# PreferredAI/cornac

Hardware: AMD Instinct MI355X
Metric: bpr_triplets_per_sec (higher is better)
Workload: dtype f32

## Files before the change

cornac_amd/csrc/bpr.hip:

```cpp
#include <algorithm>
#include <numeric>
#include <queue>

#include "common.h"
#include "rng.h"
#include "sgd_device.h"

namespace chip {

__global__ __launch_bounds__(kBlock) void bpr_det_sample_kernel(
    const uint32_t *__restrict__ pos_draw, int pos_stride, const uint32_t *__restrict__ neg_draw, int neg_stride,
    int64_t n, const int32_t *__restrict__ user_ids, const int32_t *__restrict__ indices,
    const int32_t *__restrict__ indptr, int neg_population, int32_t *__restrict__ su, int32_t *__restrict__ si,
    int32_t *__restrict__ sj, unsigned long long *__restrict__ counters) {
    const int64_t s = (int64_t)blockIdx.x * kBlock + threadIdx.x;
    bool skip = false;
    if (s < n) {
        const uint32_t ii = pos_draw[s * pos_stride];
        const uint32_t jj = neg_draw[s * neg_stride];
        const int32_t u = user_ids[ii];
        const int32_t i = indices[ii];
        const int32_t j = neg_population == CORNAC_HIP_NEG_POPULARITY ? indices[jj] : (int32_t)jj;
        skip = csr_row_contains(indices, indptr[u], indptr[u + 1], j);
        su[s] = skip ? -1 : u;
        si[s] = i;
        sj[s] = j;
    }
    const unsigned long long m = __ballot(skip);
    if (lane_id() == 0 && m) atomicAdd(&counters[1], (unsigned long long)__popcll(m));
}

template <int G, class T>
__global__ __launch_bounds__(kBlock) void bpr_det_level_kernel(const int32_t *__restrict__ su,
                                                               const int32_t *__restrict__ si,
                                                               const int32_t *__restrict__ sj, int64_t off, int cnt,
                                                               T *U, T *V, T *B, int k, T lr,
                                                               T reg, int use_bias,
                                                               unsigned long long *__restrict__ counters) {
    const int gid = (blockIdx.x * kBlock + threadIdx.x) / G;
    const int lg = threadIdx.x & (G - 1);
    const bool active = gid < cnt;
    const int64_t t = off + (active ? gid : cnt - 1);
    const int32_t u = su[t], i = si[t], j = sj[t];
    T *pu = U + (size_t)u * k, *pi = V + (size_t)i * k, *pj = V + (size_t)j * k;
    const T bi = B[i], bj = B[j];
    T score = bi - bj;
    constexpr int RMAX = 4;
    T ru[RMAX], ri[RMAX], rj[RMAX];
    const bool in_regs = k <= RMAX * G;
#pragma unroll
    for (int r = 0; r < RMAX; ++r) {
        const int f = r * G + lg;
        ru[r] = ri[r] = rj[r] = T(0);
        if (in_regs && f < k) {
            ru[r] = pu[f];
            ri[r] = pi[f];
            rj[r] = pj[f];
        }
    }
    auto ordered_add = [&](T p, int lim) { score = ordered_lane_sum_t<G>(score, p, lim); };
    if (in_regs) {
#pragma unroll
        for (int r = 0; r < RMAX; ++r) {
            const int base = r * G;
            if (base < k) ordered_add(base + lg < k ? ru[r] * (ri[r] - rj[r]) : T(0), min(G, k - base));
        }
    } else {
        for (int base = 0; base < k; base += G) {
            const int f = base + lg;
            ordered_add(f < k ? pu[f] * (pi[f] - pj[f]) : T(0), min(G, k - base));
        }
    }
    const T z = sigmoid_neg_exact_t(score);
    if (active) {
        if (in_regs) {
#pragma unroll
            for (int r = 0; r < RMAX; ++r) {
                const int f = r * G + lg;
                if (f < k) {
                    const T uf = ru[r], vi = ri[r], vj = rj[r];
                    pu[f] = uf + lr * (z * (vi - vj) - reg * uf);
                    pi[f] = vi + lr * (z * uf - reg * vi);
                    pj[f] = vj + lr * (-z * uf - reg * vj);
                }
            }
// ... 1404 lines not shown
    const int grid = di.cus * h->strata_blocks_per_cu;
    const int64_t W = (int64_t)grid * kWavesPerBlock;
    if (h->own_waves != W) h->strata_built = false;
    build_ownership(h, W);
    build_item_ranks(h);
    h->rec_u.ensure((size_t)h->nnz);
    h->rec_i.ensure((size_t)h->nnz);
    h->sptr.ensure((size_t)W * 8 + 1);
    REQUIRE(grid % 8 == 0, "the strata grid must be a multiple of the 8 XCDs");
    h->strata_claim.ensure(8 * 16);
    return grid;
}

static void strata_build_buckets(cornac_hip_bpr_t h, int grid, uint32_t key) {
    if (h->strata_built && h->strata_key_built == key) return;
    StrataArgs s;
    s.own_u = h->own_u.p; s.own_i = h->own_i.p; s.wave_ptr = h->wave_ptr.p; s.item_rank = h->item_rank.p;
    s.rec_u = h->rec_u.p; s.rec_i = h->rec_i.p; s.sptr = h->sptr.p;
    s.key = key; s.n_hot = h->strata_n_hot; s.n_waves = (int64_t)grid * kWavesPerBlock;
    h->strata_own_code.ensure((size_t)h->nnz);
    s.own_code = h->strata_own_code.p;
    if (h->strata_code_waves != h->own_waves) {
        hipLaunchKernelGGL(strata_code_kernel, dim3((unsigned)std::min<int64_t>(4096, (h->nnz + kBlock - 1) / kBlock)),
                           dim3(kBlock), 0, h->stream, s, h->nnz);
        h->strata_code_waves = h->own_waves;
    }
    hipLaunchKernelGGL(strata_bucket_kernel, dim3(grid), dim3(kBlock), 0, h->stream, s);
    HIP_CHECK(hipGetLastError());
    h->strata_built = true;
    h->strata_key_built = key;
    ++h->strata_builds;
}

static void strata_enqueue(cornac_hip_bpr_t h, int64_t n_samples, float lr, float reg, int use_bias, int flags) {
    const int grid = strata_prepare(h);
    const bool packed = h->strata_allow_pack && ((h->V.owned && h->B.owned) || h->chunk_records) &&
                        !prof_env_set("CORNAC_HIP_STRATA_NO_PACK");
    if (packed) strata_pack(h); else strata_unpack(h);
    if (!packed) h->Bpad.ensure((size_t)h->total_items * kBiasStride);
    const unsigned bgrid = (unsigned)((h->total_items + kBlock - 1) / kBlock);
    int64_t left = n_samples;
    while (left > 0) {
        const int64_t n = std::min(left, h->nnz - h->hog_offset);
        const auto first_phase = [&](int64_t s) { return (int)((8 * (__int128)s + h->nnz - 1) / h->nnz); };
        const int p_lo = first_phase(h->hog_offset), p_hi = h->hog_offset + n >= h->nnz ? 8 : first_phase(h->hog_offset + n);
        if (p_hi > p_lo) {
            uint32_t key = strata_key(h->hog_seed, h->hog_epoch / (uint32_t)std::max(1, h->strata_rehash_period));
            if (prof_env_int("CORNAC_HIP_STRATA_CONTIG", 0)) key = 0x12345u;
            strata_build_buckets(h, grid, key);
            HogArgs a;
            fill_hog_args(h, a, h->nnz, lr, reg, use_bias, CORNAC_HIP_NEG_UNIFORM, flags);
            const bool dense_bias = !packed && prof_env_int("CORNAC_HIP_STRATA_DENSE_BIAS", 0) != 0;
            a.B = dense_bias ? h->B.p : h->Bpad.p;
            a.bstride = dense_bias ? 1 : kBiasStride;
            if (packed) {
                a.V = h->VB.p;
                a.vpitch = h->vb_pitch;
                a.B = h->VB.p + h->vb_kp;
                a.bstride = h->vb_pitch;
            }
            a.rec_u = h->rec_u.p; a.rec_i = h->rec_i.p; a.rank_item = h->rank_item.p; a.sptr = h->sptr.p;
            a.strata_key = key; a.n_hot = h->strata_n_hot;
            HIP_CHECK(hipMemsetAsync(h->strata_claim.p, 0, 8 * 16 * sizeof(uint32_t), h->stream));
            if (!dense_bias && !packed)
                hipLaunchKernelGGL(bias_pad_kernel, dim3(bgrid), dim3(kBlock), 0, h->stream, h->B.p, h->Bpad.p, h->total_items);
            for (int ph = p_lo; ph < p_hi; ++ph) {
                a.phase = ph;
                a.xcd_claim = h->strata_claim.p + 16 * ph;
                h->ktimer.before(h->stream);
                hipLaunchKernelGGL(h->strata_kernel, dim3(grid), dim3(kBlock), 0, h->stream, a);
                h->ktimer.after(h->stream);
            }
            if (!dense_bias && !packed)
                hipLaunchKernelGGL(bias_unpad_kernel, dim3(bgrid), dim3(kBlock), 0, h->stream, h->Bpad.p, h->B.p, h->total_items);
            HIP_CHECK(hipGetLastError());
        }
        advance_hog_offset(h, n);
        left -= n;
    }
}

typedef void (*LdsBinKernel)(const LdsBinArgs);
constexpr int kLdsbinPresampleDefault = 0;
static LdsBinKernel pick_ldsbin_kernel(int k, bool pop, bool exch = false, bool passing = false, bool conv = false, bool pre = false) {
    if (pre) {
        if (k <= 64) return bpr_ldsbin_kernel<1, 4, false, false, 1, false, true>;
        return bpr_ldsbin_kernel<2, 2, false, false, 1, false, true>;
    }
    if (conv) {
        if (pop) {
            if (k <= 64) return bpr_ldsbin_kernel<1, 4, true, false, 1, true>;
            if (k <= 128) return bpr_ldsbin_kernel<2, 4, true, false, 1, true>;
            if (k <= 192) return bpr_ldsbin_kernel<3, 2, true, false, 1, true>;
            return bpr_ldsbin_kernel<4, 1, true, false, 1, true>;
        }
        if (k <= 64) return bpr_ldsbin_kernel<1, 4, false, false, 1, true>;
        if (k <= 128) return bpr_ldsbin_kernel<2, 4, false, false, 1, true>;
        if (k <= 192) return bpr_ldsbin_kernel<3, 2, false, false, 1, true>;
        return bpr_ldsbin_kernel<4, 1, false, false, 1, true>;
    }
    if (passing && !exch && k > 64 && k <= 128) {
#ifdef CORNAC_PROFILE
        if (prof_env_int("CORNAC_HIP_LDSBIN_UNR", 0) == 0)
#endif
            return pop ? bpr_ldsbin_kernel<2, 4, true> : bpr_ldsbin_kernel<2, 4>;
    }
    if (exch) {
        if (pop) {
            if (k <= 64) return bpr_ldsbin_kernel<1, 4, true, true>;
            if (k <= 128) return bpr_ldsbin_kernel<2, 2, true, true>;
            if (k <= 192) return bpr_ldsbin_kernel<3, 2, true, true>;
            return bpr_ldsbin_kernel<4, 1, true, true>;
        }
        if (k <= 64) return bpr_ldsbin_kernel<1, 4, false, true>;
        if (k <= 128) return bpr_ldsbin_kernel<2, 2, false, true>;
        if (k <= 192) return bpr_ldsbin_kernel<3, 2, false, true>;
        return bpr_ldsbin_kernel<4, 1, false, true>;
    }
    if (pop) {
        if (k <= 64) return bpr_ldsbin_kernel<1, 4, true>;
        if (k <= 128) return bpr_ldsbin_kernel<2, 2, true>;
        if (k <= 192) return bpr_ldsbin_kernel<3, 2, true>;
        return bpr_ldsbin_kernel<4, 1, true>;
    }
#ifdef CORNAC_PROFILE
    if (k <= 64) switch (prof_env_int("CORNAC_HIP_LDSBIN_UNR", 0)) {
        case 1: return bpr_ldsbin_kernel<1, 1>;
        case 2: return bpr_ldsbin_kernel<1, 2>;
        case 8: return bpr_ldsbin_kernel<1, 8>;
        default: break;
    }
    else if (k <= 128) switch (prof_env_int("CORNAC_HIP_LDSBIN_UNR", 0)) {
        case 3: return bpr_ldsbin_kernel<2, 3>;
        case 4: return bpr_ldsbin_kernel<2, 4>;
        case 22: return bpr_ldsbin_kernel<2, 2, false, false, 2>;
        case 32: return bpr_ldsbin_kernel<2, 3, false, false, 2>;
        case 42: return bpr_ldsbin_kernel<2, 4, false, false, 2>;
        default: break;
    }
#endif
    if (k <= 64) return bpr_ldsbin_kernel<1, 4>;
    if (k <= 128) return bpr_ldsbin_kernel<2, 2>;
    if (k <= 192) return bpr_ldsbin_kernel<3, 2>;
    return bpr_ldsbin_kernel<4, 1>;
}

constexpr size_t kLbLdsBudget = 96 * 1024;
constexpr size_t kLbLdsExclusive = 82 * 1024;
static size_t ldsbin_lds_bytes(int cap, int k, int waves = kLbWaves) {
    const int kp = ((k + kWave - 1) / kWave) * kWave;
    return ((size_t)cap * (kp + 5) + 1) * sizeof(float) + (size_t)waves * 3 * kWave * sizeof(int32_t);
}

struct LbPlan {
    int bins = 0, block = kLbBlock, cap = 0;
    size_t lds = 0;
    bool passing = false;
};
static LbPlan ldsbin_plan(cornac_hip_bpr_t h) {
    LbPlan pl;
    const int cus = device_info(h->device).cus;
    if (h->cv_blocks) {
        if (h->k > 256) return pl;
        const int waves = h->lb_pass_waves;
        const size_t budget = (size_t)h->lb_pass_kb << 10;
        const int kp = ((h->k + kWave - 1) / kWave) * kWave;
        const size_t fixed = sizeof(float) + (size_t)waves * 3 * kWave * sizeof(int32_t);
        if (budget <= fixed) return pl;
        const int64_t cap_lds = (int64_t)((budget - fixed) / ((size_t)(kp + 5) * sizeof(float)));
        const int64_t cap_min = std::max<int64_t>(h->lb_min_candidates, 16);
        if (cap_lds < cap_min) return pl;
        int64_t bins = (h->n_items + cap_lds - 1) / cap_lds;
        const int64_t more = std::min<int64_t>(h->n_items / (cap_min + cap_min / 3), (int64_t)2 * cus * h->cv_blocks);
        bins = std::max(bins, more);
        bins = std::max<int64_t>(1, (bins + h->cv_blocks - 1) / h->cv_blocks) * h->cv_blocks;
        const int64_t cap = (h->n_items + bins - 1) / bins;
        if (cap > cap_lds || bins > (int64_t(1) << 22) || bins * cap >= (int64_t(1) << 31)) return pl;
        pl.bins = (int)bins;
        pl.cap = (int)cap;
        pl.block = waves * kWave;
        pl.lds = ldsbin_lds_bytes((int)cap, h->k, waves);
        pl.passing = true;
        return pl;
    }
    if (h->k > 256 || h->nnz < (int64_t)cus * kLbWaves * kWave) return pl;
    const int res_waves = prof_env_int("CORNAC_HIP_LDSBIN_RES_WAVES", kLbWaves);
    for (int rounds = prof_env_int("CORNAC_HIP_LDSBIN_MIN_ROUNDS", 1); rounds <= h->lb_max_rounds; ++rounds) {
        const int64_t bins = (int64_t)cus * rounds;
        const int64_t cap = (h->n_items + bins - 1) / bins;
        if (cap < h->lb_min_candidates) return pl;
        if (ldsbin_lds_bytes((int)cap, h->k, res_waves) <= (size_t)prof_env_int("CORNAC_HIP_LDSBIN_BUDGET_KB", (int)(kLbLdsBudget >> 10)) << 10) {
            pl.bins = (int)bins;
            pl.cap = (int)cap;
            pl.block = res_waves * kWave;
            pl.lds = std::max(ldsbin_lds_bytes((int)cap, h->k, res_waves), (size_t)prof_env_int("CORNAC_HIP_LDSBIN_EXCL_KB", (int)(kLbLdsExclusive >> 10)) << 10);
            return pl;
        }
    }
    if (!h->lb_pass_enable || (double)h->nnz * 100.0 < (double)h->n_items * h->lb_pass_min_draws_x100) return pl;
    const int waves = prof_env_int("CORNAC_HIP_LDSBIN_PASS_WAVES", h->lb_pass_waves);
    const size_t budget = (size_t)prof_env_int("CORNAC_HIP_LDSBIN_PASS_KB", h->lb_pass_kb) << 10;
    const int kp = ((h->k + kWave - 1) / kWave) * kWave;
    const size_t fixed = sizeof(float) + (size_t)waves * 3 * kWave * sizeof(int32_t);
    if (budget <= fixed) return pl;
    int64_t cap = (int64_t)((budget - fixed) / ((size_t)(kp + 5) * sizeof(float)));
    if (cap < h->lb_min_candidates) return pl;
    int64_t bins = (h->n_items + cap - 1) / cap;
    bins = ((bins + cus - 1) / cus) * cus;
    cap = (h->n_items + bins - 1) / bins;
    if (cap < h->lb_min_candidates || bins > (int64_t(1) << 22)) return pl;
    pl.bins = (int)bins;
    pl.cap = (int)cap;
    pl.block = waves * kWave;
    pl.lds = ldsbin_lds_bytes((int)cap, h->k, waves);
    pl.passing = true;
    return pl;
}

static bool ldsbin_can_run(cornac_hip_bpr_t h, int64_t n_samples, int neg_population) {
    if (neg_population == CORNAC_HIP_NEG_POPULARITY && h->neg_pop_n) return false;
    const LbPlan pl = ldsbin_plan(h);
    return pl.bins > 0 && (!pl.passing || n_samples * 4 >= h->nnz);
}

static void ldsbin_build(cornac_hip_bpr_t h) {
    const LbPlan plan = ldsbin_plan(h);
    const int bins = plan.bins;
    if (h->lb_built && h->lb_bins == bins && h->lb_block == plan.block && h->lb_lds_bytes == plan.lds) return;
// ... 766 lines not shown
```

cornac_amd/csrc/bpr_ldsbin.inc:

```


namespace chip {

constexpr int kLbBlock = 1024;
constexpr int kLbWaves = kLbBlock / kWave;
constexpr int32_t kLbHot = (int32_t)0x80000000;
constexpr int kLbMaxExchanges = 32;
constexpr int kLbMaxRanges = 8;

struct LdsBinExchange {
    float *base;
    float *bucket;
    float *keep;
    unsigned int *arrive;
    const unsigned int *landed;
    unsigned int *applied;
    long long bucket_stride, keep_stride;
    long long nt;
    int n_ex, rule;
};

struct LdsBinArgs {
    const int32_t *cptr, *cusers;
    const int32_t *rank_item;
// ... 316 lines not shown
        uint32_t run = 0;
        for (uint32_t g0 = 0; g0 < n_groups; g0 += kWave) {
            const uint32_t g = g0 + lane;
            uint32_t v = g < n_groups ? cum[g + 1] : 0u;
#pragma unroll
            for (int o = 1; o < kWave; o <<= 1) {
                const uint32_t t = __shfl_up(v, o, kWave);
                if (lane >= o) v += t;
            }
            if (g < n_groups) cum[g + 1] = run + v;
            run += __shfl(v, kWave - 1, kWave);
        }
        if (lane == 0) {
            cum[0] = 0;
            *sh_next_tile = 0;
            *sh_cold_mass = run;
            *sh_nslots = (n_groups && item[n_groups - 1] == -1) ? n_groups - 1 : n_groups;
        }
    }
    __syncthreads();
}

template <bool POP>
__device__ __forceinline__ LdsBinDraw ldsbin_draw(const LdsBinArgs &a, const LdsBinCtx &c, uint32_t local, bool in_range) {
    LdsBinDraw d;
    d.in_range = in_range;
    uint32_t w[4];
    philox4x32_10(d.in_range ? local : 0u, c.b, a.epoch, 0x20u, (uint32_t)a.seed, (uint32_t)(a.seed >> 32), w);
    const uint32_t r_pos = lemire_bounded2(w[0], w[1], c.n_draws, c.th_draw);
    uint32_t s_j, excl = 0, excl_lo = 0xffffffffu;
    if (r_pos < c.cold_mass) {
        uint32_t lo = 0, hi = c.n_slots;
        while (hi - lo > 1) {
            const uint32_t mid = (lo + hi) >> 1;
            if (c.cum[mid] <= r_pos) lo = mid; else hi = mid;
        }
        d.u = a.cusers[c.cp[lo] + (int32_t)(r_pos - c.cum[lo])];
        d.ei = (int32_t)lo;
        s_j = c.n_slots > 1 ? lemire_bounded2(w[2], w[3], c.n_slots - 1, c.th_slot1) : 0u;
        if (c.n_slots > 1 && s_j >= lo) ++s_j;
        excl_lo = c.cum[lo];
        excl = c.cum[lo + 1] - excl_lo;
    } else {
        const uint32_t h = c.hot_lo + (r_pos - c.cold_mass);
        d.u = a.hot_u[h];
        d.ei = a.hot_i[h] | kLbHot;
        s_j = lemire_bounded2(w[2], w[3], c.n_slots, c.th_slot);
    }
    if (POP) {
        const uint32_t m = c.n_draws - excl;
        uint32_t r_neg = (uint32_t)(((uint64_t)w[2] * m) >> 32);
        if (r_neg >= excl_lo) r_neg += excl;
        if (m == 0) {
            d.j = c.item[d.ei] & ~kLbHot;
            d.ej = d.ei;
        } else if (r_neg < c.cold_mass) {
            uint32_t lo = 0, hi = c.n_slots;
            while (hi - lo > 1) {
                const uint32_t mid = (lo + hi) >> 1;
                if (c.cum[mid] <= r_neg) lo = mid; else hi = mid;
            }
            d.j = c.item[lo];
            d.ej = (int32_t)lo;
        } else {
            d.j = a.hot_i[c.hot_lo + (r_neg - c.cold_mass)];
            d.ej = d.j | kLbHot;
        }
        return d;
    }
    const int32_t itj = c.item[s_j];
    d.j = itj & ~kLbHot;
    d.ej = itj < 0 ? itj : (int32_t)s_j;
    return d;
}

__device__ __forceinline__ void ldsbin_launch_range(const LdsBinArgs &a, uint32_t n_draws, uint32_t n_waves, uint32_t &d_lo,
                                                    uint32_t &d_hi, uint32_t &tile_w, uint32_t &n_tiles) {
    d_lo = (uint32_t)(((unsigned __int128)n_draws * a.s_begin) / a.nnz);
    d_hi = a.s_begin + a.n >= a.nnz ? n_draws : (uint32_t)(((unsigned __int128)n_draws * (a.s_begin + a.n)) / a.nnz);
    tile_w = (d_hi - d_lo) < 8u * n_waves * kWave ? 32u : 64u;
    n_tiles = (d_hi - d_lo + tile_w - 1) / tile_w;
}

template <int R, int UNR, bool POP = false, bool EXCH = false, int PF = 1, bool CONV = false, bool PRE = false>
__global__ __launch_bounds__(kLbBlock) void bpr_ldsbin_kernel(const LdsBinArgs a) {
    constexpr int G = kWave, KP = G * R, NREF = 2 * UNR;
    extern __shared__ float lb_smem[];
    float *const rows = lb_smem;
    float *const bias = rows + (size_t)a.cap * KP;
    int32_t *const item = reinterpret_cast<int32_t *>(bias + a.cap);
    int32_t *const cp = item + a.cap;
    uint32_t *const cum = reinterpret_cast<uint32_t *>(cp + a.cap);
    int *const lock = reinterpret_cast<int *>(cum + a.cap + 1);
    int32_t(*const stage)[3][kWave] = reinterpret_cast<int32_t(*)[3][kWave]>(lock + a.cap);
    const int wave = threadIdx.x >> 6, lane = lane_id();
    const uint32_t n_waves = blockDim.x >> 6;
    uint32_t b = blockIdx.x;
    const uint32_t nb = (uint32_t)a.n_bins;
    float *cvV = nullptr, *cvB = nullptr;
    if (CONV) {
        const uint32_t r = blockIdx.x / (uint32_t)a.conv_bpb, o = blockIdx.x - r * (uint32_t)a.conv_bpb;
        b = (uint32_t)a.conv_first[r] + o;
        cvV = a.conv_rows[r] + (size_t)o * (size_t)a.cap * (size_t)a.k;
        cvB = a.conv_rows[r] + (size_t)a.conv_bpb * (size_t)a.cap * (size_t)a.k + (size_t)o * (size_t)a.cap;
    }
    const uint32_t n_groups = ((uint32_t)a.n_items + nb - 1) / nb;
#ifdef CORNAC_PROFILE
    if (a.wg_clock && threadIdx.x == 0) a.wg_clock[2 * b] = wall_clock64();
#endif
    __shared__ uint32_t sh_nslots, sh_cold_mass, sh_next_tile;
    __shared__ uint32_t sh_ex_done[kLbMaxExchanges], sh_ex_applied[kLbWaves];
    __shared__ int sh_ex_lock[kLbWaves];
    if (EXCH) {
        if (threadIdx.x < kLbMaxExchanges) sh_ex_done[threadIdx.x] = 0;
        if (threadIdx.x < kLbWaves) {
            sh_ex_applied[threadIdx.x] = 0;
            sh_ex_lock[threadIdx.x] = 0;
        }
    }
    ldsbin_build_tables(a, b, nb, n_groups, item, cp, cum, lock, &sh_nslots, &sh_cold_mass, &sh_next_tile);
    const uint32_t n_slots = sh_nslots, cold_mass = sh_cold_mass;
    const uint32_t hot_lo = a.hot_off[b], hot_share = a.hot_off[b + 1] - hot_lo;
    const uint32_t n_draws = n_slots ? cold_mass + hot_share : 0u;
    const uint32_t th_draw = n_draws ? lemire_thresh(n_draws) : 0u, th_slot = n_slots ? lemire_thresh(n_slots) : 0u,
                   th_slot1 = n_slots > 1 ? lemire_thresh(n_slots - 1) : 0u;
    bool inb[R];
#pragma unroll
    for (int r = 0; r < R; ++r) inb[r] = lane + G * r < a.k;
    {
        constexpr int NL = R <= 2 ? 4 : 2;
        for (uint32_t s0 = wave; s0 < n_slots; s0 += n_waves * NL) {
            float t[NL][R], tb[NL];
            int32_t its[NL];
#pragma unroll
            for (int q = 0; q < NL; ++q) {
                const uint32_t sq = s0 + (uint32_t)q * n_waves;
                its[q] = sq < n_slots ? item[sq] : -1;
                const size_t it = (size_t)(its[q] >= 0 ? its[q] : 0);
                const float *pv = CONV ? cvV + (size_t)(its[q] >= 0 ? sq : 0u) * a.k : a.V + it * a.k;
                const float *pb = CONV ? cvB + (its[q] >= 0 ? sq : 0u) : a.B + it;
#pragma unroll
                for (int r = 0; r < R; ++r) t[q][r] = (its[q] >= 0 && inb[r]) ? pv[lane + G * r] : 0.f;
                tb[q] = (its[q] >= 0 && lane == 0) ? *pb : 0.f;
            }
#pragma unroll
            for (int q = 0; q < NL; ++q) {
                if (its[q] < 0) continue;
                const uint32_t sq = s0 + (uint32_t)q * n_waves;
#pragma unroll
                for (int r = 0; r < R; ++r) rows[(size_t)sq * KP + lane + G * r] = t[q][r];
                if (lane == 0) bias[sq] = tb[q];
            }
        }
    }
    __syncthreads();
    unsigned int n_correct = 0, n_skipped = 0;
    if (!PRE && n_slots == 0 && wave == 0 && lane == 0 && a.s_begin == 0) n_skipped = cold_mass + hot_share;
    uint32_t d_lo, d_hi, tile_w, n_tiles;
    ldsbin_launch_range(a, n_draws, n_waves, d_lo, d_hi, tile_w, n_tiles);
    const LdsBinCtx ctx{item, cp, cum, b, n_slots, cold_mass, hot_lo, n_draws, th_draw, th_slot, th_slot1};
    typedef LdsBinDraw Draws;
    auto draw_tile = [&](uint32_t tile) {
        const uint32_t local = d_lo + tile * tile_w + lane;
        return ldsbin_draw<POP>(a, ctx, local, tile < n_tiles && (uint32_t)lane < tile_w && local < d_hi);
    };
    auto member_word = [&](const Draws &d) -> uint32_t {
        return (a.bitmap && !LB_ABLATE(1)) ? a.bitmap[(size_t)d.u * a.bm_words + (d.j >> 5)] : 0u;
    };
    auto member_bounds = [&](const Draws &d, int32_t &lo, int32_t &hi) {
        lo = hi = 0;
        if (!a.bitmap && !LB_ABLATE(1) && d.in_range) {
            lo = a.indptr[d.u];
            hi = a.indptr[d.u + 1];
        }
    };
    auto claim_tile = [&]() -> uint32_t {
        uint32_t t = 0;
        if (lane == 0) t = atomicAdd(&sh_next_tile, 1u);
        return (uint32_t)__builtin_amdgcn_readfirstlane((int)t);
    };
    const uint32_t ex_per = EXCH ? n_tiles / (uint32_t)a.ex.n_ex : 0u;
    const uint32_t ex_parts = ex_per < n_waves ? ex_per : n_waves;
    auto ex_landed_upto = [&](int from, int below) -> int {
        int e = from;
        if (lane == 0)
            while (e < below && __hip_atomic_load(a.ex.landed + e, __ATOMIC_RELAXED, __HIP_MEMORY_SCOPE_SYSTEM) != 0u) ++e;
        return __builtin_amdgcn_readfirstlane(e);
    };
    auto ex_duty = [&](uint32_t t) {
        if (!EXCH || ex_parts == 0u || t >= n_tiles) return;
        const uint32_t q = t / ex_per, part = t - q * ex_per;
        if (q == 0u || q >= (uint32_t)a.ex.n_ex || part >= ex_parts) return;
        const int e = (int)q - 1;
        if (lane == 0)
            while (atomicCAS(&sh_ex_lock[part], 0, 1) != 0) __builtin_amdgcn_s_sleep(2);
        __builtin_amdgcn_fence(__ATOMIC_ACQUIRE, "workgroup");
        const int e_lo = (int)sh_ex_applied[part];
        const int e_hi = ex_landed_upto(e_lo, e);
        if (e_hi > e_lo) __builtin_amdgcn_fence(__ATOMIC_ACQUIRE, "agent");
        constexpr int NB = R == 1 ? 4 : 2;
        if (!LB_ABLATE(64)) {
            for (uint32_t s = part; s < n_slots; s += ex_parts) {
                const int32_t it = item[s];
                if (it >= 0)
                    ex_row_duty<R>(a.ex, a.V, a.B, a.k, it, rows + (size_t)s * KP, bias + s, lock + s, e_lo, e_hi, e, lane, inb, a.counters + 3);
            }
        } else
        for (uint32_t s0 = part; s0 < n_slots; s0 += ex_parts * NB) {
            int32_t its[NB];
            float *lrow[NB], *lbias[NB];
            int *llock[NB];
#pragma unroll
            for (int q = 0; q < NB; ++q) {
                const uint32_t s = s0 + (uint32_t)q * ex_parts;
                const uint32_t sc = s < n_slots ? s : s0;
                const int32_t it = item[sc];
                its[q] = (s < n_slots && it >= 0) ? it : -1;
                lrow[q] = rows + (size_t)sc * KP;
                lbias[q] = bias + sc;
                llock[q] = lock + sc;
            }
            ex_rows_duty<R, NB>(a.ex, a.k, its, lrow, lbias, llock, e_lo, e_hi, e, lane, inb, a.counters + 3);
        }
        if (part == 0u)
            for (uint32_t hr = b; hr < (uint32_t)a.n_hot; hr += nb)
                ex_row_duty<R>(a.ex, a.V, a.B, a.k, a.rank_item[hr], nullptr, nullptr, nullptr, e_lo, e_hi, e, lane, inb, a.counters + 3);
        asm volatile("s_waitcnt vmcnt(0)" ::: "memory");
        if (lane == 0) {
            sh_ex_applied[part] = (uint32_t)e_hi;
            __builtin_amdgcn_fence(__ATOMIC_RELEASE, "workgroup");
            __hip_atomic_store(&sh_ex_lock[part], 0, __ATOMIC_RELAXED, __HIP_MEMORY_SCOPE_WORKGROUP);
            if (atomicAdd(&sh_ex_done[e], 1u) == ex_parts - 1u)
                __hip_atomic_fetch_add(a.ex.arrive + e, 1u, __ATOMIC_RELAXED, __HIP_MEMORY_SCOPE_SYSTEM);
        }
    };
    auto train_tile = [&](const int nvalid) __attribute__((always_inline)) {
        float u_nx[PF][UNR][R];
        int32_t tu_nx[PF][UNR];
        auto request_users = [&](float (&ub)[UNR][R], int32_t (&tub)[UNR], int t0) {
#pragma unroll
            for (int q = 0; q < UNR; ++q) {
                const int sl = t0 + q < nvalid ? t0 + q : (t0 < nvalid ? t0 : 0);
                tub[q] = __builtin_amdgcn_readfirstlane(stage[wave][0][sl]);
#pragma unroll
                for (int r = 0; r < R; ++r)
                    ub[q][r] = !inb[r] || LB_ABLATE(4) ? 0.f
                               : LB_ABLATE(8)          ? load_f32_fresh(a.U + (size_t)tub[q] * a.k + lane + G * r)
                                                       : __builtin_nontemporal_load(a.U + (size_t)tub[q] * a.k + lane + G * r);
            }
        };
        auto step = [&](float (&ub)[UNR][R], int32_t (&tub)[UNR], int t0) {
            float u_[UNR][R], v_[NREF][R], bv[NREF];
            float *pu[UNR];
            int32_t ref[NREF];
            bool act[UNR];
#pragma unroll
            for (int q = 0; q < UNR; ++q) {
                act[q] = t0 + q < nvalid;
                const int sl = act[q] ? t0 + q : t0;
                ref[2 * q] = __builtin_amdgcn_readfirstlane(stage[wave][1][sl]);
                ref[2 * q + 1] = __builtin_amdgcn_readfirstlane(stage[wave][2][sl]);
                pu[q] = a.U + (size_t)tub[q] * a.k + lane;
#pragma unroll
                for (int r = 0; r < R; ++r) u_[q][r] = ub[q][r];
            }
            if (t0 + PF * UNR < nvalid) request_users(ub, tub, t0 + PF * UNR);
#pragma unroll
            for (int c = 0; c < NREF; ++c) {
                if (ref[c] < 0) {
                    const int32_t it = ref[c] & ~kLbHot;
#pragma unroll
                    for (int r = 0; r < R; ++r) v_[c][r] = inb[r] ? load_f32_fresh(a.V + (size_t)it * a.k + lane + G * r) : 0.f;
                    bv[c] = load_f32_fresh(a.B + it);
                } else {
#pragma unroll
                    for (int r = 0; r < R; ++r) v_[c][r] = rows[(size_t)ref[c] * KP + lane + G * r];
                    bv[c] = bias[ref[c]];
                }
            }
            float du[UNR][R], zq[UNR];
#pragma unroll
            for (int q = 0; q < UNR; ++q) {
                float part = 0.f;
#pragma unroll
                for (int r = 0; r < R; ++r) part += u_[q][r] * (v_[2 * q][r] - v_[2 * q + 1][r]);
                const float score = (bv[2 * q] - bv[2 * q + 1]) + (LB_ABLATE(256) ? part : LB_ABLATE(1024) ? group_sum<G>(part) : wave_sum_dpp(part));
                const float z = LB_ABLATE(512) ? 0.5f + 1e-3f * score : sigmoid_neg_fast(score);
                zq[q] = z;
#pragma unroll
                for (int r = 0; r < R; ++r) du[q][r] = a.lr * (z * (v_[2 * q][r] - v_[2 * q + 1][r]) - a.reg * u_[q][r]);
                if (act[q] && lane == 0) n_correct += z < .5f ? 1u : 0u;
            }
#pragma unroll
            for (int q = 0; q < UNR; ++q) {
                if (!act[q] || LB_ABLATE(2)) continue;
#pragma unroll
                for (int r = 0; r < R; ++r)
                    if (inb[r]) {
                        if (LB_ABLATE(8)) store_f32_agent(pu[q] + G * r, u_[q][r] + du[q][r]);
                        else if (LB_ABLATE(16)) pu[q][G * r] = u_[q][r] + du[q][r];
                        else atomic_add_f32(pu[q] + G * r, du[q][r]);
                    }
            }
#pragma unroll
            for (int c = 0; c < NREF; ++c) {
                const int q = c >> 1;
                if (!act[q] || LB_ABLATE(2)) continue;
                const float zs = (c & 1) ? -zq[q] : zq[q];
                if (ref[c] < 0) {
                    const int32_t it = ref[c] & ~kLbHot;
#pragma unroll
                    for (int r = 0; r < R; ++r)
                        if (inb[r]) atomic_add_f32(a.V + (size_t)it * a.k + lane + G * r, a.lr * (zs * u_[q][r] - a.reg * v_[c][r]));
                    if (a.use_bias && lane == 0) atomic_add_f32(a.B + it, a.lr * (zs - a.reg * bv[c]));
                    continue;
                }
                const int s = ref[c];
                if (LB_ABLATE(32)) continue;
                if (!EXCH && LB_ABLATE(2048)) {
#pragma unroll
                    for (int r = 0; r < R; ++r)
                        atomicAdd(rows + (size_t)s * KP + lane + G * r, a.lr * (zs * u_[q][r] - a.reg * v_[c][r]));
                    if (a.use_bias && lane == 0) atomicAdd(bias + s, a.lr * (zs - a.reg * bv[c]));
                    continue;
                }
                const bool owned = LB_ABLATE(128) ? false : lds_row_lock(&lock[s], lane, a.counters + 3);
#pragma unroll
                for (int r = 0; r < R; ++r) {
                    float *pv = rows + (size_t)s * KP + lane + G * r;
                    const float v = *pv;
                    *pv = v + a.lr * (zs * u_[q][r] - a.reg * v);
                }
                if (a.use_bias && lane == 0) {
                    const float bb = bias[s];
                    bias[s] = bb + a.lr * (zs - a.reg * bb);
                }
                if (!LB_ABLATE(128)) lds_row_unlock(&lock[s], lane, owned);
            }
        };
        if (nvalid) request_users(u_nx[0], tu_nx[0], 0);
        if (PF == 2 && UNR < nvalid) request_users(u_nx[PF - 1], tu_nx[PF - 1], UNR);
        for (int t0 = 0; t0 < nvalid; t0 += PF * UNR) {
            step(u_nx[0], tu_nx[0], t0);
            if (PF == 2 && t0 + UNR < nvalid) step(u_nx[PF - 1], tu_nx[PF - 1], t0 + UNR);
        }
    };
    if constexpr (PRE) {
        const size_t pool0 = (size_t)a.pre_base[b];
        int32_t rec[3] = {0, 0, 0};
        uint32_t cnt = 0;
        auto fetch = [&](uint32_t t) {
            if (t < n_tiles) {
                const size_t o = pool0 + t;
                cnt = a.pre_cnt[o];
#pragma unroll
                for (int q = 0; q < 3; ++q) rec[q] = a.pre_rec[(o * 3 + q) * kWave + lane];
            }
        };
        uint32_t tB = n_tiles ? claim_tile() : 0u;
        fetch(tB);
        while (tB < n_tiles) {
            const int nvalid = __builtin_amdgcn_readfirstlane((int)cnt);
#pragma unroll
            for (int q = 0; q < 3; ++q) stage[wave][q][lane] = rec[q];
            __builtin_amdgcn_fence(__ATOMIC_ACQ_REL, "wavefront");
            __builtin_amdgcn_wave_barrier();
            tB = claim_tile();
            fetch(tB);
            train_tile(nvalid);
            __builtin_amdgcn_wave_barrier();
        }
    } else {
    uint32_t tB = n_tiles ? claim_tile() : 0u;
    Draws dB = n_tiles ? draw_tile(tB) : Draws{0, 0, 0, 0, false};
    if (n_tiles) ex_duty(tB);
    uint32_t tA = n_tiles ? claim_tile() : 0u;
    Draws dA = n_tiles ? draw_tile(tA) : dB;
    if (n_tiles) ex_duty(tA);
    uint32_t wordB = (n_tiles && dB.in_range) ? member_word(dB) : 0u;
    int32_t rowB_lo, rowB_hi;
    member_bounds(dB, rowB_lo, rowB_hi);
    while (tB < n_tiles) {
        bool skip = (wordB >> (dB.j & 31)) & 1u;
        if (!a.bitmap && !LB_ABLATE(1) && dB.in_range) skip = csr_row_contains(a.indices, rowB_lo, rowB_hi, dB.j);
        const bool valid = dB.in_range && !skip;
        const unsigned long long mask = __ballot(valid);
        n_skipped += (dB.in_range && !valid) ? 1u : 0u;
        if (valid) {
            const int pos = __popcll(mask & ((1ull << lane) - 1ull));
            stage[wave][0][pos] = dB.u;
            stage[wave][1][pos] = dB.ei;
            stage[wave][2][pos] = dB.ej;
        }
        __builtin_amdgcn_fence(__ATOMIC_ACQ_REL, "wavefront");
        __builtin_amdgcn_wave_barrier();
        const int nvalid = __popcll(mask);
        dB = dA;
        tB = tA;
        wordB = dB.in_range ? member_word(dB) : 0u;
        member_bounds(dB, rowB_lo, rowB_hi);
        tA = claim_tile();
        dA = draw_tile(tA);
        ex_duty(tA);
        train_tile(nvalid);
        __builtin_amdgcn_wave_barrier();
    }
    }
    __syncthreads();
    if (EXCH) {
        const int n_ex = a.ex.n_ex;
        const int landed_hi = ex_landed_upto(0, n_ex - 1);
        if (landed_hi > 0) __builtin_amdgcn_fence(__ATOMIC_ACQUIRE, "agent");
        for (int e = ex_parts ? n_ex - 1 : 0; e < n_ex; ++e) {
            const bool first = e == (ex_parts ? n_ex - 1 : 0);
            for (uint32_t s = wave; s < n_slots; s += n_waves) {
                const int32_t it = item[s];
                if (it < 0) continue;
                const int lo = ex_parts ? (int)sh_ex_applied[s % ex_parts] : 0;
                const int hi = ex_parts ? (landed_hi > lo ? landed_hi : lo) : 0;
                ex_row_duty<R>(a.ex, a.V, a.B, a.k, it, rows + (size_t)s * KP, bias + s, nullptr, first ? lo : hi, hi, e, lane, inb, a.counters + 3);
                if (lane == 0) a.ex.applied[it] = (unsigned int)hi;
            }
            if (wave == 0)
                for (uint32_t hr = b; hr < (uint32_t)a.n_hot; hr += nb) {
                    const int32_t it = a.rank_item[hr];
                    const int lo = ex_parts ? (int)sh_ex_applied[0] : 0;
                    const int hi = ex_parts ? (landed_hi > lo ? landed_hi : lo) : 0;
                    ex_row_duty<R>(a.ex, a.V, a.B, a.k, it, nullptr, nullptr, nullptr, first ? lo : hi, hi, e, lane, inb, a.counters + 3);
                    if (lane == 0) a.ex.applied[it] = (unsigned int)hi;
                }
            asm volatile("s_waitcnt vmcnt(0)" ::: "memory");
            __syncthreads();
            if (threadIdx.x == 0) __hip_atomic_fetch_add(a.ex.arrive + e, 1u, __ATOMIC_RELAXED, __HIP_MEMORY_SCOPE_SYSTEM);
        }
    }
    for (uint32_t s = wave; s < n_slots; s += n_waves) {
        const int32_t it = item[s];
        if (it >= 0) {
            float *pv = CONV ? cvV + (size_t)s * a.k : a.V + (size_t)it * a.k;
#pragma unroll
            for (int r = 0; r < R; ++r)
                if (inb[r]) pv[lane + G * r] = rows[(size_t)s * KP + lane + G * r];
            if (lane == 0) *(CONV ? cvB + s : a.B + it) = bias[s];
        }
    }
#pragma unroll
    for (int o = 32; o > 0; o >>= 1) {
        n_correct += __shfl_xor(n_correct, o, kWave);
        n_skipped += __shfl_xor(n_skipped, o, kWave);
    }
    if (lane == 0) {
        if (n_correct) atomicAdd(&a.counters[0], (unsigned long long)n_correct);
        if (n_skipped) atomicAdd(&a.counters[1], (unsigned long long)n_skipped);
    }
#ifdef CORNAC_PROFILE
    __syncthreads();
    if (a.wg_clock && threadIdx.x == 0) a.wg_clock[2 * b + 1] = wall_clock64();
#endif
}

struct LdsTileBaseArgs {
    const uint32_t *cold, *hot_off;
    uint32_t *base;
    uint64_t s_begin, n, nnz;
    int32_t n_bins;
    uint32_t n_waves;
};

__global__ __launch_bounds__(kLbBlock) void ldsbin_tilebase_kernel(const LdsTileBaseArgs t) {
    __shared__ uint32_t carry;
    if (threadIdx.x == 0) carry = 0;
    __syncthreads();
    const int wave = threadIdx.x >> 6, lane = lane_id();
    (void)wave;
    for (int32_t b0 = 0; b0 < t.n_bins; b0 += kLbBlock) {
        const int32_t b = b0 + (int32_t)threadIdx.x;
        uint32_t tiles = 0;
        if (b < t.n_bins) {
            const uint32_t n_draws = t.cold[b] + (t.hot_off[b + 1] - t.hot_off[b]);
            const uint32_t d_lo = (uint32_t)(((unsigned __int128)n_draws * t.s_begin) / t.nnz);
            const uint32_t d_hi = t.s_begin + t.n >= t.nnz ? n_draws : (uint32_t)(((unsigned __int128)n_draws * (t.s_begin + t.n)) / t.nnz);
            const uint32_t tile_w = (d_hi - d_lo) < 8u * t.n_waves * kWave ? 32u : 64u;
            tiles = (d_hi - d_lo + tile_w - 1) / tile_w;
        }
        __shared__ uint32_t wsum[kLbWaves];
        uint32_t v = tiles;
#pragma unroll
// ... 276 lines not shown
```

Measured before the change: 3.432 billion.

## Add full-k specialization and a cold-triplet steady path in ldsbin BPR kernel

Adds a FULLK template flag, chosen when k exactly equals 64*R, so the per-lane bounds predicates become compile-time true. Within each tile, triplets whose item and negative rows are both cold (LDS-resident, not hot) are ordered first. A branch-free steady-state step loop then handles them in whole UNR groups, skipping the hot-row global-memory paths and the per-step validity checks. The remaining hot or leftover triplets use the original generic path. This costs more template instantiations and code size. The stage reordering and the inserted waitcnt also change the processing order within a tile.

New measurement: 3.377 billion. 0.984x the previous value.

```diff
diff --git a/cornac_amd/csrc/bpr.hip b/cornac_amd/csrc/bpr.hip
--- a/cornac_amd/csrc/bpr.hip
+++ b/cornac_amd/csrc/bpr.hip
@@ -1,6 +1,7 @@
 #include <algorithm>
 #include <numeric>
 #include <queue>
+#include <type_traits>
 
 #include "common.h"
 #include "rng.h"
@@ -1571,6 +1572,7 @@
 
 typedef void (*LdsBinKernel)(const LdsBinArgs);
 constexpr int kLdsbinPresampleDefault = 0;
+#define LB_FULLK(R, ...) (k == 64 * (R) ? bpr_ldsbin_kernel<R, __VA_ARGS__, true> : bpr_ldsbin_kernel<R, __VA_ARGS__, false>)
 static LdsBinKernel pick_ldsbin_kernel(int k, bool pop, bool exch = false, bool passing = false, bool conv = false, bool pre = false) {
     if (pre) {
         if (k <= 64) return bpr_ldsbin_kernel<1, 4, false, false, 1, false, true>;
@@ -1578,13 +1580,13 @@
     }
     if (conv) {
         if (pop) {
-            if (k <= 64) return bpr_ldsbin_kernel<1, 4, true, false, 1, true>;
-            if (k <= 128) return bpr_ldsbin_kernel<2, 4, true, false, 1, true>;
+            if (k <= 64) return LB_FULLK(1, 4, true, false, 1, true, false);
+            if (k <= 128) return LB_FULLK(2, 4, true, false, 1, true, false);
             if (k <= 192) return bpr_ldsbin_kernel<3, 2, true, false, 1, true>;
             return bpr_ldsbin_kernel<4, 1, true, false, 1, true>;
         }
-        if (k <= 64) return bpr_ldsbin_kernel<1, 4, false, false, 1, true>;
-        if (k <= 128) return bpr_ldsbin_kernel<2, 4, false, false, 1, true>;
+        if (k <= 64) return LB_FULLK(1, 4, false, false, 1, true, false);
+        if (k <= 128) return LB_FULLK(2, 4, false, false, 1, true, false);
         if (k <= 192) return bpr_ldsbin_kernel<3, 2, false, false, 1, true>;
         return bpr_ldsbin_kernel<4, 1, false, false, 1, true>;
     }
@@ -1592,47 +1594,48 @@
 #ifdef CORNAC_PROFILE
         if (prof_env_int("CORNAC_HIP_LDSBIN_UNR", 0) == 0)
 #endif
-            return pop ? bpr_ldsbin_kernel<2, 4, true> : bpr_ldsbin_kernel<2, 4>;
+            return pop ? LB_FULLK(2, 4, true, false, 1, false, false) : LB_FULLK(2, 4, false, false, 1, false, false);
     }
     if (exch) {
         if (pop) {
-            if (k <= 64) return bpr_ldsbin_kernel<1, 4, true, true>;
-            if (k <= 128) return bpr_ldsbin_kernel<2, 2, true, true>;
+            if (k <= 64) return LB_FULLK(1, 4, true, true, 1, false, false);
+            if (k <= 128) return LB_FULLK(2, 2, true, true, 1, false, false);
             if (k <= 192) return bpr_ldsbin_kernel<3, 2, true, true>;
             return bpr_ldsbin_kernel<4, 1, true, true>;
         }
-        if (k <= 64) return bpr_ldsbin_kernel<1, 4, false, true>;
-        if (k <= 128) return bpr_ldsbin_kernel<2, 2, false, true>;
+        if (k <= 64) return LB_FULLK(1, 4, false, true, 1, false, false);
+        if (k <= 128) return LB_FULLK(2, 2, false, true, 1, false, false);
         if (k <= 192) return bpr_ldsbin_kernel<3, 2, false, true>;
         return bpr_ldsbin_kernel<4, 1, false, true>;
     }
     if (pop) {
-        if (k <= 64) return bpr_ldsbin_kernel<1, 4, true>;
-        if (k <= 128) return bpr_ldsbin_kernel<2, 2, true>;
+        if (k <= 64) return LB_FULLK(1, 4, true, false, 1, false, false);
+        if (k <= 128) return LB_FULLK(2, 2, true, false, 1, false, false);
         if (k <= 192) return bpr_ldsbin_kernel<3, 2, true>;
         return bpr_ldsbin_kernel<4, 1, true>;
     }
 #ifdef CORNAC_PROFILE
     if (k <= 64) switch (prof_env_int("CORNAC_HIP_LDSBIN_UNR", 0)) {
-        case 1: return bpr_ldsbin_kernel<1, 1>;
-        case 2: return bpr_ldsbin_kernel<1, 2>;
-        case 8: return bpr_ldsbin_kernel<1, 8>;
+        case 1: return LB_FULLK(1, 1, false, false, 1, false, false);
+        case 2: return LB_FULLK(1, 2, false, false, 1, false, false);
+        case 8: return LB_FULLK(1, 8, false, false, 1, false, false);
         default: break;
     }
     else if (k <= 128) switch (prof_env_int("CORNAC_HIP_LDSBIN_UNR", 0)) {
-        case 3: return bpr_ldsbin_kernel<2, 3>;
-        case 4: return bpr_ldsbin_kernel<2, 4>;
-        case 22: return bpr_ldsbin_kernel<2, 2, false, false, 2>;
-        case 32: return bpr_ldsbin_kernel<2, 3, false, false, 2>;
-        case 42: return bpr_ldsbin_kernel<2, 4, false, false, 2>;
+        case 3: return LB_FULLK(2, 3, false, false, 1, false, false);
+        case 4: return LB_FULLK(2, 4, false, false, 1, false, false);
+        case 22: return LB_FULLK(2, 2, false, false, 2, false, false);
+        case 32: return LB_FULLK(2, 3, false, false, 2, false, false);
+        case 42: return LB_FULLK(2, 4, false, false, 2, false, false);
         default: break;
     }
 #endif
-    if (k <= 64) return bpr_ldsbin_kernel<1, 4>;
-    if (k <= 128) return bpr_ldsbin_kernel<2, 2>;
+    if (k <= 64) return LB_FULLK(1, 4, false, false, 1, false, false);
+    if (k <= 128) return LB_FULLK(2, 2, false, false, 1, false, false);
     if (k <= 192) return bpr_ldsbin_kernel<3, 2>;
     return bpr_ldsbin_kernel<4, 1>;
 }
+#undef LB_FULLK
 
 constexpr size_t kLbLdsBudget = 96 * 1024;
 constexpr size_t kLbLdsExclusive = 82 * 1024;
diff --git a/cornac_amd/csrc/bpr_ldsbin.inc b/cornac_amd/csrc/bpr_ldsbin.inc
--- a/cornac_amd/csrc/bpr_ldsbin.inc
+++ b/cornac_amd/csrc/bpr_ldsbin.inc
@@ -422,9 +422,10 @@
     n_tiles = (d_hi - d_lo + tile_w - 1) / tile_w;
 }
 
-template <int R, int UNR, bool POP = false, bool EXCH = false, int PF = 1, bool CONV = false, bool PRE = false>
+template <int R, int UNR, bool POP = false, bool EXCH = false, int PF = 1, bool CONV = false, bool PRE = false, bool FULLK = false>
 __global__ __launch_bounds__(kLbBlock) void bpr_ldsbin_kernel(const LdsBinArgs a) {
     constexpr int G = kWave, KP = G * R, NREF = 2 * UNR;
+    constexpr bool kSteady = FULLK && PF == 1 && !PRE;
     extern __shared__ float lb_smem[];
     float *const rows = lb_smem;
     float *const bias = rows + (size_t)a.cap * KP;
@@ -466,7 +467,7 @@
                    th_slot1 = n_slots > 1 ? lemire_thresh(n_slots - 1) : 0u;
     bool inb[R];
 #pragma unroll
-    for (int r = 0; r < R; ++r) inb[r] = lane + G * r < a.k;
+    for (int r = 0; r < R; ++r) inb[r] = FULLK || lane + G * r < a.k;
     {
         constexpr int NL = R <= 2 ? 4 : 2;
         for (uint32_t s0 = wave; s0 < n_slots; s0 += n_waves * NL) {
@@ -574,7 +575,7 @@
                 __hip_atomic_fetch_add(a.ex.arrive + e, 1u, __ATOMIC_RELAXED, __HIP_MEMORY_SCOPE_SYSTEM);
         }
     };
-    auto train_tile = [&](const int nvalid) __attribute__((always_inline)) {
+    auto train_tile = [&](const int nvalid, const int n_cold) __attribute__((always_inline)) {
         float u_nx[PF][UNR][R];
         int32_t tu_nx[PF][UNR];
         auto request_users = [&](float (&ub)[UNR][R], int32_t (&tub)[UNR], int t0) {
@@ -589,14 +590,15 @@
                                                        : __builtin_nontemporal_load(a.U + (size_t)tub[q] * a.k + lane + G * r);
             }
         };
-        auto step = [&](float (&ub)[UNR][R], int32_t (&tub)[UNR], int t0) {
+        auto step = [&](auto steady, float (&ub)[UNR][R], int32_t (&tub)[UNR], int t0) {
+            constexpr bool ST = decltype(steady)::value;
             float u_[UNR][R], v_[NREF][R], bv[NREF];
             float *pu[UNR];
             int32_t ref[NREF];
             bool act[UNR];
 #pragma unroll
             for (int q = 0; q < UNR; ++q) {
-                act[q] = t0 + q < nvalid;
+                act[q] = ST || t0 + q < nvalid;
                 const int sl = act[q] ? t0 + q : t0;
                 ref[2 * q] = __builtin_amdgcn_readfirstlane(stage[wave][1][sl]);
                 ref[2 * q + 1] = __builtin_amdgcn_readfirstlane(stage[wave][2][sl]);
@@ -604,10 +606,10 @@
 #pragma unroll
                 for (int r = 0; r < R; ++r) u_[q][r] = ub[q][r];
             }
-            if (t0 + PF * UNR < nvalid) request_users(ub, tub, t0 + PF * UNR);
+            if (ST || t0 + PF * UNR < nvalid) request_users(ub, tub, t0 + PF * UNR);
 #pragma unroll
             for (int c = 0; c < NREF; ++c) {
-                if (ref[c] < 0) {
+                if (!ST && ref[c] < 0) {
                     const int32_t it = ref[c] & ~kLbHot;
 #pragma unroll
                     for (int r = 0; r < R; ++r) v_[c][r] = inb[r] ? load_f32_fresh(a.V + (size_t)it * a.k + lane + G * r) : 0.f;
@@ -647,7 +649,7 @@
                 const int q = c >> 1;
                 if (!act[q] || LB_ABLATE(2)) continue;
                 const float zs = (c & 1) ? -zq[q] : zq[q];
-                if (ref[c] < 0) {
+                if (!ST && ref[c] < 0) {
                     const int32_t it = ref[c] & ~kLbHot;
 #pragma unroll
                     for (int r = 0; r < R; ++r)
@@ -678,11 +680,20 @@
                 if (!LB_ABLATE(128)) lds_row_unlock(&lock[s], lane, owned);
             }
         };
-        if (nvalid) request_users(u_nx[0], tu_nx[0], 0);
+        int t_gen = 0;
+        if constexpr (kSteady) {
+            const int n_steady = n_cold - n_cold % UNR;
+            if (n_steady > 0) {
+                request_users(u_nx[0], tu_nx[0], 0);
+                __builtin_amdgcn_s_waitcnt(0x0F70);
+                for (; t_gen < n_steady; t_gen += UNR) step(std::true_type{}, u_nx[0], tu_nx[0], t_gen);
+            }
+        }
+        if (t_gen == 0 && nvalid) request_users(u_nx[0], tu_nx[0], 0);
         if (PF == 2 && UNR < nvalid) request_users(u_nx[PF - 1], tu_nx[PF - 1], UNR);
-        for (int t0 = 0; t0 < nvalid; t0 += PF * UNR) {
-            step(u_nx[0], tu_nx[0], t0);
-            if (PF == 2 && t0 + UNR < nvalid) step(u_nx[PF - 1], tu_nx[PF - 1], t0 + UNR);
+        for (int t0 = t_gen; t0 < nvalid; t0 += PF * UNR) {
+            step(std::false_type{}, u_nx[0], tu_nx[0], t0);
+            if (PF == 2 && t0 + UNR < nvalid) step(std::false_type{}, u_nx[PF - 1], tu_nx[PF - 1], t0 + UNR);
         }
     };
     if constexpr (PRE) {
@@ -707,7 +718,7 @@
             __builtin_amdgcn_wave_barrier();
             tB = claim_tile();
             fetch(tB);
-            train_tile(nvalid);
+            train_tile(nvalid, 0);
             __builtin_amdgcn_wave_barrier();
         }
     } else {
@@ -724,10 +735,13 @@
         bool skip = (wordB >> (dB.j & 31)) & 1u;
         if (!a.bitmap && !LB_ABLATE(1) && dB.in_range) skip = csr_row_contains(a.indices, rowB_lo, rowB_hi, dB.j);
         const bool valid = dB.in_range && !skip;
-        const unsigned long long mask = __ballot(valid);
+        const bool cold = valid && dB.ei >= 0 && dB.ej >= 0;
+        const unsigned long long mask = __ballot(valid), cmask = __ballot(cold);
+        const int n_cold = __popcll(cmask);
         n_skipped += (dB.in_range && !valid) ? 1u : 0u;
         if (valid) {
-            const int pos = __popcll(mask & ((1ull << lane) - 1ull));
+            const unsigned long long below = (1ull << lane) - 1ull;
+            const int pos = cold ? __popcll(cmask & below) : n_cold + __popcll(mask & ~cmask & below);
             stage[wave][0][pos] = dB.u;
             stage[wave][1][pos] = dB.ei;
             stage[wave][2][pos] = dB.ej;
@@ -742,7 +756,7 @@
         tA = claim_tile();
         dA = draw_tile(tA);
         ex_duty(tA);
-        train_tile(nvalid);
+        train_tile(nvalid, n_cold);
         __builtin_amdgcn_wave_barrier();
     }
     }
```
